# jolibrain/joliGEN

Measured on AMD Instinct MI355X. Metric: train images/sec at 256x256 (DDPM UNet step), higher is better.
Workload: dtype bf16; 1 GPU; palette_model DDPM, efficient UNet unet_mha ngf64 mults[1,2,4,8] res_blocks[2,2,2,2] mid-attn 16x32, 256x256, batch 32/GPU, inpainting synthetic masks, AdamW+EMA, iter_size 1 (example_ddpm_noglasses2glasses.json + SURVEY Appendix C overrides); global_batch=32, per_gpu_batch=32, image_size=256, efficient=True, parallelism=dp1, n_ranks_seen=1

## Files before the change

joligen_amd/csrc/capi.hip:

```cpp
#include "common.h"

extern "C" int jg_version(void) { return 100; }

extern "C" const char* jg_strerror(int code) {
  switch (code) {
    case JG_OK: return "ok";
    case JG_ERR_BAD_ARG: return "bad argument (null pointer, misaligned leading dimension or unsupported shape)";
    case JG_ERR_UNSUPPORTED: return "unsupported configuration";
    case JG_ERR_LAUNCH: return "HIP launch failed";
    default: return "unknown error";
  }
}

#include <atomic>
#include <cstdlib>
#include <cstring>
#include <mutex>

namespace {
struct TuneDef { const char* env; int dflt; };
const TuneDef kTune[JG_TUNE_COUNT] = {
    {"JG_HALO_CFG", 0}, {"JG_WGRAD_HALO_CFG", 0}, {"JG_CONV_VARIANT", 6}, {"JG_WGRAD_VARIANT", 4}, {"JG_SINKHORN_GENERIC", 0},
    {"JG_CONV1X1", 1}, {"JG_GN_REVERSE", 1}, {"JG_HALO_DBG", 0}, {"JG_PERSIST64", 1}, {"JG_HALO_PIPE", 1}, {"JG_WGRAD_PIPE", 1}, {"JG_CONV_SPLITK", 1}, {"JG_CONV_SMALL_TILE", 1}, {"JG_GN_FUSED", 1}, {"JG_GN_FUSED_CAP", 256}, {"JG_GN_FUSED_DBG", 0}, {"JG_GN_FUSED_SLEEP", 4}, {"JG_WGRAD_LDS_PAD", 0},
    {"JG_LN_BWD_CAP", 256}, {"JG_DW_BWD_CAP", 512}, {"JG_DW_BWD_PPT", 8}, {"JG_CONV_KXK", 1}, {"JG_CONV_RING", 1}, {"JG_WGRAD_DEEP", 1}, {"JG_WGRAD_SW", 0}, {"JG_DETERMINISTIC", 0}, {"JG_WGRAD_GROUP_BLOCKS", 1024}, {"JG_SGEMM_SPLIT", 0}, {"JG_WGRAD_BIG", 1}, {"JG_DW_RUN", 1}};
std::atomic<int> g_tune[JG_TUNE_COUNT];
std::once_flag g_tune_once;
void tune_init() {
  for (int i = 0; i < JG_TUNE_COUNT; ++i) {
    const char* e = getenv(kTune[i].env);
    g_tune[i].store(e ? atoi(e) : kTune[i].dflt, std::memory_order_relaxed);
  }
}
}

namespace {
thread_local const char* g_last_kernel = "";
}
void jg_note_kernel(const char* name) { g_last_kernel = name ? name : ""; }
extern "C" const char* jg_last_kernel(void) { return g_last_kernel; }

int jg_tune(int which) {
  std::call_once(g_tune_once, tune_init);
  return g_tune[which].load(std::memory_order_relaxed);
}

extern "C" int jg_set_tuning(const char* name, int value) {
  if (!name) return JG_ERR_BAD_ARG;
  std::call_once(g_tune_once, tune_init);
  for (int i = 0; i < JG_TUNE_COUNT; ++i)
    if (!strcmp(name, kTune[i].env)) {
      g_tune[i].store(value, std::memory_order_relaxed);
      return JG_OK;
    }
  return JG_ERR_BAD_ARG;
}

extern "C" int jg_get_tuning(const char* name) {
  if (!name) return -1;
  for (int i = 0; i < JG_TUNE_COUNT; ++i)
    if (!strcmp(name, kTune[i].env)) return jg_tune(i);
  return -1;
}
```

joligen_amd/csrc/common.h:

```cpp
#pragma once
#include <hip/hip_runtime.h>
#include <stdint.h>

#include "../../include/jg355.h"

typedef _Float16 f16_t;
typedef __bf16 bf16_t;
typedef _Float16 f16x8 __attribute__((ext_vector_type(8)));
typedef __bf16 bf16x8 __attribute__((ext_vector_type(8)));
typedef float f32x4 __attribute__((ext_vector_type(4)));

#define JG_WAVE 64

enum JgTune { JG_TUNE_HALO_CFG = 0, JG_TUNE_WGRAD_HALO_CFG, JG_TUNE_CONV_VARIANT, JG_TUNE_WGRAD_VARIANT, JG_TUNE_SINKHORN_GENERIC,
              JG_TUNE_CONV1X1, JG_TUNE_GN_REVERSE, JG_TUNE_HALO_DBG, JG_TUNE_PERSIST64, JG_TUNE_HALO_PIPE, JG_TUNE_WGRAD_PIPE, JG_TUNE_CONV_SPLITK, JG_TUNE_CONV_SMALL_TILE, JG_TUNE_GN_FUSED, JG_TUNE_GN_FUSED_CAP, JG_TUNE_GN_FUSED_DBG, JG_TUNE_GN_FUSED_SLEEP, JG_TUNE_WGRAD_LDS_PAD,
              JG_TUNE_LN_BWD_CAP, JG_TUNE_DW_BWD_CAP, JG_TUNE_DW_BWD_PPT, JG_TUNE_CONV_KXK, JG_TUNE_CONV_RING, JG_TUNE_WGRAD_DEEP, JG_TUNE_WGRAD_SW, JG_TUNE_DETERMINISTIC, JG_TUNE_WGRAD_GROUP_BLOCKS, JG_TUNE_SGEMM_SPLIT, JG_TUNE_WGRAD_BIG, JG_TUNE_DW_RUN, JG_TUNE_COUNT };
int jg_tune(int which);
void jg_note_kernel(const char* name);

#define JG_CHECK_LAUNCH()                          \
  do {                                             \
    if (hipGetLastError() != hipSuccess) return JG_ERR_LAUNCH; \
  } while (0)

template <typename T> __device__ __forceinline__ float to_f32(T v) { return (float)v; }
template <typename T> __device__ __forceinline__ T from_f32(float v) { return (T)v; }

template <typename T> __device__ __forceinline__ T bits_to(uint16_t b) { return __builtin_bit_cast(T, b); }
template <typename T> __device__ __forceinline__ uint16_t to_bits(T v) { return __builtin_bit_cast(uint16_t, v); }

template <typename T> __device__ __forceinline__ void unpack8(const uint4& v, float* f) {
  const uint32_t w[4] = {v.x, v.y, v.z, v.w};
#pragma unroll
  for (int i = 0; i < 4; ++i) {
    f[2 * i] = to_f32(bits_to<T>((uint16_t)(w[i] & 0xffffu)));
    f[2 * i + 1] = to_f32(bits_to<T>((uint16_t)(w[i] >> 16)));
  }
}
template <typename T> __device__ __forceinline__ uint4 pack8(const float* f) {
  uint32_t w[4];
#pragma unroll
  for (int i = 0; i < 4; ++i) {
    w[i] = (uint32_t)to_bits<T>(from_f32<T>(f[2 * i])) | ((uint32_t)to_bits<T>(from_f32<T>(f[2 * i + 1])) << 16);
  }
  return make_uint4(w[0], w[1], w[2], w[3]);
}
template <typename T> __device__ __forceinline__ uint2 pack4(float a, float b, float c, float d) {
  uint2 r;
  r.x = (uint32_t)to_bits<T>(from_f32<T>(a)) | ((uint32_t)to_bits<T>(from_f32<T>(b)) << 16);
  r.y = (uint32_t)to_bits<T>(from_f32<T>(c)) | ((uint32_t)to_bits<T>(from_f32<T>(d)) << 16);
  return r;
}
template <typename T> __device__ __forceinline__ void unpack4(const uint2& v, float* f) {
  f[0] = to_f32(bits_to<T>((uint16_t)(v.x & 0xffffu)));
  f[1] = to_f32(bits_to<T>((uint16_t)(v.x >> 16)));
  f[2] = to_f32(bits_to<T>((uint16_t)(v.y & 0xffffu)));
  f[3] = to_f32(bits_to<T>((uint16_t)(v.y >> 16)));
}

template <typename T> struct Mfma;
template <> struct Mfma<f16_t> {
  static __device__ __forceinline__ f32x4 run(const uint4& a, const uint4& b, f32x4 c) {
    return __builtin_amdgcn_mfma_f32_16x16x32_f16(__builtin_bit_cast(f16x8, a), __builtin_bit_cast(f16x8, b), c, 0, 0, 0);
  }
};
template <> struct Mfma<bf16_t> {
  static __device__ __forceinline__ f32x4 run(const uint4& a, const uint4& b, f32x4 c) {
    return __builtin_amdgcn_mfma_f32_16x16x32_bf16(__builtin_bit_cast(bf16x8, a), __builtin_bit_cast(bf16x8, b), c, 0, 0, 0);
  }
};

template <typename T> __device__ __forceinline__ uint4 ldg16(const T* ptr, bool ok) {
  uint4 v = *reinterpret_cast<const uint4*>(ptr);
  v.x = ok ? v.x : 0u;
  v.y = ok ? v.y : 0u;
  v.z = ok ? v.z : 0u;
  v.w = ok ? v.w : 0u;
  return v;
}

__device__ __forceinline__ float sigmoid_fast(float u) { return __builtin_amdgcn_rcpf(1.0f + __expf(-u)); }
__device__ __forceinline__ float silu_f(float u) { return u * sigmoid_fast(u); }
__device__ __forceinline__ float silu_grad_f(float u) {
  const float s = sigmoid_fast(u);
  return s * (1.0f + u * (1.0f - s));
}

template <int ACT> __device__ __forceinline__ float act_f(float u) {
  if (ACT == JG_ACT_SILU) return silu_f(u);
  if (ACT == JG_ACT_RELU) return fmaxf(u, 0.f);
  if (ACT == JG_ACT_LRELU) return u > 0.f ? u : 0.2f * u;
  return u;
}
template <int ACT> __device__ __forceinline__ float act_grad_f(float u) {
  if (ACT == JG_ACT_SILU) return silu_grad_f(u);
  if (ACT == JG_ACT_RELU) return u > 0.f ? 1.f : 0.f;
  if (ACT == JG_ACT_LRELU) return u > 0.f ? 1.f : 0.2f;
  return 1.f;
}
__device__ __forceinline__ float act_grad_rt(float u, int act) {
  return act == JG_ACT_SILU ? silu_grad_f(u) : act == JG_ACT_RELU ? (u > 0.f ? 1.f : 0.f) : act == JG_ACT_LRELU ? (u > 0.f ? 1.f : 0.2f) : 1.f;
}

#define JG_DISPATCH_ACT(act, ...)                          \
  do {                                                     \
    if ((act) == JG_ACT_SILU) { constexpr int ACT = JG_ACT_SILU; __VA_ARGS__ }        \
    else if ((act) == JG_ACT_RELU) { constexpr int ACT = JG_ACT_RELU; __VA_ARGS__ }   \
    else if ((act) == JG_ACT_LRELU) { constexpr int ACT = JG_ACT_LRELU; __VA_ARGS__ } \
    else { constexpr int ACT = JG_ACT_NONE; __VA_ARGS__ }                              \
  } while (0)

__device__ __forceinline__ float wave_sum(float v) {
#pragma unroll
  for (int o = 32; o > 0; o >>= 1) v += __shfl_xor(v, o);
  return v;
}
__device__ __forceinline__ float wave_max(float v) {
#pragma unroll
  for (int o = 32; o > 0; o >>= 1) v = fmaxf(v, __shfl_xor(v, o));
  return v;
}

#define JG_DISPATCH_DTYPE(dtype, ...)                 \
  do {                                                \
    if ((dtype) == JG_F16) {                          \
      typedef f16_t T;                                \
      __VA_ARGS__                                     \
    } else if ((dtype) == JG_BF16) {                  \
      typedef bf16_t T;                               \
      __VA_ARGS__                                     \
    } else {                                          \
      return JG_ERR_BAD_ARG;                          \
    }                                                 \
  } while (0)
```

joligen_amd/csrc/conv_p64.hip:

```cpp
#include "conv_params.h"
#include "conv_epilogue.h"

namespace {

constexpr int HW_ = 18;
constexpr int HALO_CH = HW_ * HW_ * 8;
constexpr int W_CH = 64 * 9 * 8;
constexpr int REGION = HALO_CH / 4;
constexpr int A_RD = (REGION + 63) / 64;

__device__ uint4 jg_p64_zero_page = {0u, 0u, 0u, 0u};

__device__ __forceinline__ void glds16(const void* gsrc, unsigned lds_dst) {
  unsigned keep;
  asm volatile("s_mov_b32 %0, m0\n\ts_mov_b32 m0, %2\n\ts_nop 0\n\tglobal_load_lds_dwordx4 %1, off\n\ts_mov_b32 m0, %0"
               : "=&s"(keep) : "v"(gsrc), "s"(lds_dst) : "memory");
}
template <int N> __device__ __forceinline__ void wait_vmcnt() { asm volatile("s_waitcnt vmcnt(%0)" ::"n"(N) : "memory"); }

struct TileRef { int b, oh0, ow0, sp; };

template <typename T>
__global__ __launch_bounds__(512, 1) void conv3x3_p64_kernel(ConvP p, int nsp, int Gs, int tilesN) {
  __shared__ uint4 sm[W_CH + 2 * HALO_CH + 16];
  const int tid = threadIdx.x, lane = tid & 63;
  const int wave = __builtin_amdgcn_readfirstlane(tid >> 6);
  const int g = wave >> 2, w = wave & 3;
  const int nb = blockIdx.x % tilesN, stream = blockIdx.x / tilesN;
  const int n0 = nb * 64;
  const int per = (nsp + Gs - 1) / Gs;
  const int ntl = stream * per < nsp ? (nsp - stream * per < per ? nsp - stream * per : per) : 0;
  const int tw = p.W >> 4, th = p.H >> 4;

  const T* __restrict__ x = (const T*)p.x;
  const T* __restrict__ wt = (const T*)p.w;
  const T* zp = reinterpret_cast<const T*>(&jg_p64_zero_page);
  typedef __attribute__((address_space(3))) char* lds_cptr;
  const unsigned lds0 = (unsigned)(size_t)(lds_cptr)(char*)&sm[0];
  char* smc = reinterpret_cast<char*>(&sm[0]);
  const unsigned hbyte = (W_CH + g * HALO_CH) * 16;

  auto tile_of = [&](int k) {
    TileRef t;
    t.sp = stream * per + k;
    t.ow0 = (t.sp % tw) << 4;
    t.oh0 = ((t.sp / tw) % th) << 4;
    t.b = t.sp / (tw * th);
    return t;
  };

  auto issue_halo = [&](const TileRef& t) {
    const long org = (((long)t.b * p.H + t.oh0) * p.W + t.ow0) * p.ldx;
    int lane_v = lane;
    asm volatile("" : "+v"(lane_v));
#pragma unroll
    for (int rd = 0; rd < A_RD; ++rd) {
      const int q = rd * 64 + lane_v;
      if (q < REGION) {
        const int pos = w * REGION + q;
        const int hp = pos >> 3, cpos = pos & 7;
        const int hy = (hp * 3641) >> 16, hx = hp - hy * HW_;
        const int kc = cpos ^ ((hx >> 1) & 7);
        const int ih = t.oh0 - 1 + hy, iw = t.ow0 - 1 + hx;
        const bool ok = (unsigned)ih < (unsigned)p.H && (unsigned)iw < (unsigned)p.W;
        const T* src = ok ? x + org + ((long)(hy - 1) * p.W + (hx - 1)) * p.ldx + kc * 8 : zp;
        glds16(src, lds0 + hbyte + (w * REGION + rd * 64) * 16);
      }
    }
  };

  {
    const int row = tid >> 3, cpos = tid & 7;
    const int kc = cpos ^ ((row >> 1) & 7);
    const bool ok = n0 + row < p.N;
    const T* src0 = wt + (long)(n0 + row) * p.ldw + kc * 8;
#pragma unroll
    for (int tap = 0; tap < 9; ++tap) glds16(ok ? src0 + tap * 64 : zp, lds0 + (tap * 512 + wave * 64) * 16);
  }
  if (g == 0 && ntl > 0) issue_halo(tile_of(0));

  const int l15 = lane & 15, lk = lane >> 4;
  float* sbias = reinterpret_cast<float*>(smc + (W_CH + 2 * HALO_CH) * 16);
  if (tid < 64) sbias[tid] = (p.bias && n0 + tid < p.N) ? p.bias[n0 + tid] : 0.f;

  int bfrag[4];
#pragma unroll
  for (int j = 0; j < 4; ++j) {
    const int row = j * 16 + l15;
    bfrag[j] = row * 128 + ((lk ^ ((row >> 1) & 7)) << 4);
  }
  int afrag[3];
#pragma unroll
  for (int s3 = 0; s3 < 3; ++s3) {
    const int hx = jg_pixperm(l15) + s3;
    afrag[s3] = ((w * 4) * HW_ + hx) * 128 + ((lk ^ ((hx >> 1) & 7)) << 4);
  }

  f32x4 acc[4][4];
  T* y = (T*)p.y;
  const T* res = (p.dbg & 32) ? nullptr : (const T*)p.res;
  uint2 rraw[4][4];
  auto load_res = [&](const TileRef& t) {
    const long m0 = ((long)t.b * p.H + t.oh0 + w * 4) * p.W + t.ow0 + jg_pixperm(l15);
#pragma unroll
    for (int i = 0; i < 4; ++i)
#pragma unroll
      for (int j = 0; j < 4; ++j)
        rraw[i][j] = *reinterpret_cast<const uint2*>(res + (m0 + (long)i * p.W) * p.ldres + n0 + lk * 4 + j * 16);
  };
  float s1[4][4], s2[4][4];
#pragma unroll
  for (int j = 0; j < 4; ++j)
#pragma unroll
    for (int q = 0; q < 4; ++q) s1[j][q] = s2[j][q] = 0.f;
  int stat_b = -1;
  auto flush_stats = [&]() {
    if (stat_b < 0 || !p.stats) return;
    float* dst = p.stats + (((long)stat_b * p.nslots + (blockIdx.x * 8 + wave) % p.nslots) * p.ldstats + n0) * 2;
#pragma unroll
    for (int j = 0; j < 4; ++j)
#pragma unroll
      for (int q = 0; q < 4; ++q) {
        float a = s1[j][q], b = s2[j][q];
#pragma unroll
        for (int o = 1; o < 16; o <<= 1) {
          a += __shfl_xor(a, o);
          b += __shfl_xor(b, o);
        }
        if (l15 == 0 && !(p.dbg & 64)) {
          atomicAdd(dst + (j * 16 + lk * 4 + q) * 2, a);
          atomicAdd(dst + (j * 16 + lk * 4 + q) * 2 + 1, b);
        }
        s1[j][q] = s2[j][q] = 0.f;
      }
  };
  wait_vmcnt<0>();
  __syncthreads();

  for (int ph = 0; ph <= ntl; ++ph) {
    if ((ph & 1) == g) {
      if (ph < ntl) {
        if (res) {
          if (ph < 2) load_res(tile_of(ph));
          const float rs = p.res_scale / p.alpha;
#pragma unroll
          for (int j = 0; j < 4; ++j)
#pragma unroll
            for (int i = 0; i < 4; ++i) {
              float rf[4];
              unpack4<T>(rraw[i][j], rf);
              acc[j][i] = (f32x4){rs * rf[0], rs * rf[1], rs * rf[2], rs * rf[3]};
            }
        } else {
#pragma unroll
          for (int j = 0; j < 4; ++j)
#pragma unroll
            for (int i = 0; i < 4; ++i) acc[j][i] = (f32x4){0.f, 0.f, 0.f, 0.f};
        }
        if (!(p.dbg & 2)) {
          const char* hb = smc + hbyte;
#pragma unroll
          for (int tap = 0; tap < 9; ++tap) {
            const int r = tap / 3, s3 = tap % 3;
            asm volatile("" ::: "memory");
#pragma unroll
            for (int sub = 0; sub < 2; ++sub) {
              if (sub) asm volatile("" ::: "memory");
              uint4 fa[4], fb[4];
              const int a0 = afrag[s3] ^ (sub * 64);
#pragma unroll
              for (int i = 0; i < 4; ++i) fa[i] = *reinterpret_cast<const uint4*>(hb + a0 + (i + r) * (HW_ * 128));
#pragma unroll
              for (int j = 0; j < 4; ++j) fb[j] = *reinterpret_cast<const uint4*>(smc + tap * 8192 + (bfrag[j] ^ (sub * 64)));
#pragma unroll
              for (int j = 0; j < 4; ++j)
#pragma unroll
                for (int i = 0; i < 4; ++i) acc[j][i] = Mfma<T>::run(fb[j], fa[i], acc[j][i]);
            }
          }
        }
      }
    } else {
      const int kt = ph - 1;
      const bool drain = kt >= 0 && kt < ntl && !(p.dbg & 1);
      const TileRef t = tile_of(drain ? kt : 0);
      const long mrow0 = ((long)t.b * p.H + t.oh0 + w * 4) * p.W + t.ow0 + jg_pixperm(l15);
      const bool fetch = ph + 1 < ntl && !(p.dbg & 4);
      if (fetch) issue_halo(tile_of(ph + 1));
      if (drain) {
        if (t.b != stat_b) {
          flush_stats();
          stat_b = t.b;
        }
        T* ybase = y + mrow0 * p.ldy + n0 + lk * 4;
        const long ystep = (long)p.W * p.ldy;
#pragma unroll
        for (int j = 0; j < 4; ++j) {
          const float4 bj = *reinterpret_cast<const float4*>(sbias + j * 16 + lk * 4);
          const float bq[4] = {bj.x, bj.y, bj.z, bj.w};
#pragma unroll
          for (int i = 0; i < 4; ++i) {
            float v[4];
#pragma unroll
            for (int q = 0; q < 4; ++q) v[q] = p.alpha * acc[j][i][q] + bq[q];
#pragma unroll
            for (int q = 0; q < 4; ++q) {
              s1[j][q] += v[q];
              s2[j][q] += v[q] * v[q];
            }
            if (!(p.dbg & 8)) *reinterpret_cast<uint2*>(ybase + i * ystep + j * 16) = pack4<T>(v[0], v[1], v[2], v[3]);
          }
        }
      }
      if (res && ph + 1 < ntl) {
        load_res(tile_of(ph + 1));
        wait_vmcnt<16>();
      } else {
        wait_vmcnt<0>();
      }
    }
    asm volatile("s_waitcnt lgkmcnt(0)" ::: "memory");
    __builtin_amdgcn_s_barrier();
  }
  flush_stats();
}

}

bool jg_conv_p64_try(int dtype, const ConvP& p0, int nbatch, hipStream_t st) {
  int mode = jg_tune(JG_TUNE_PERSIST64);
  if (!mode) return false;
  if (mode == 1 && p0.res) return false;
  if (mode == -1) mode = 1;
  ConvP p = p0;
  p.dbg = jg_tune(JG_TUNE_HALO_DBG);
  if (nbatch != 1 || p.R != 3 || p.S != 3 || p.pad != 1 || p.stride != 1 || p.out_f32) return false;
  if (p.Cin != 64 || p.N % 64 || (p.H & 15) || (p.W & 15) || p.H != p.Ho || p.W != p.Wo) return false;
  if (p.x_up || p.y_pool || p.res_up || p.reflect || (p.stats && p.stats_mode != 0) || p.alpha == 0.f) return false;
  if ((long)p.B * p.H * p.W * p.ldx >= (1L << 31) || (long)p.N * p.ldw >= (1L << 31)) return false;
  const int tilesN = p.N / 64;
  const int nsp = p.B * (p.H >> 4) * (p.W >> 4);
  if ((mode == 1 && nsp < 1024) || tilesN > 4) return false;
  int Gs = 256 / tilesN;
  if (mode >= 2 && Gs > mode) Gs = mode;
  if (Gs > nsp) Gs = nsp;
  const int grid = Gs * tilesN;
  jg_note_kernel("conv3x3_p64_kernel");
  if (dtype == JG_F16) hipLaunchKernelGGL((conv3x3_p64_kernel<f16_t>), dim3(grid), dim3(512), 0, st, p, nsp, Gs, tilesN);
  else if (dtype == JG_BF16) hipLaunchKernelGGL((conv3x3_p64_kernel<bf16_t>), dim3(grid), dim3(512), 0, st, p, nsp, Gs, tilesN);
  else return false;
  return true;
}
```

joligen_amd/csrc/mfma_pipe.h:

```cpp
#pragma once
#include <type_traits>
#include "common.h"

typedef unsigned u32x4 __attribute__((ext_vector_type(4)));

#define JG_MF_(MN, i) MN " %[c" #i "], %[b], %[a" #i "], %[c" #i "]\n\t"
#define JG_RD_(k) "ds_read_b128 %[d" #k "], %[p] offset:%[o" #k "]\n\t"
#define JG_C8_(c) [c0] "+v"(c[0]), [c1] "+v"(c[1]), [c2] "+v"(c[2]), [c3] "+v"(c[3]), [c4] "+v"(c[4]), [c5] "+v"(c[5]), [c6] "+v"(c[6]), [c7] "+v"(c[7])
#define JG_A8_(a) [a0] "v"(a[0]), [a1] "v"(a[1]), [a2] "v"(a[2]), [a3] "v"(a[3]), [a4] "v"(a[4]), [a5] "v"(a[5]), [a6] "v"(a[6]), [a7] "v"(a[7])
#define JG_C4_(c) [c0] "+v"(c[0]), [c1] "+v"(c[1]), [c2] "+v"(c[2]), [c3] "+v"(c[3])
#define JG_A4_(a) [a0] "v"(a[0]), [a1] "v"(a[1]), [a2] "v"(a[2]), [a3] "v"(a[3])

#define JG_G8R4_(MN)                                                                                                                  \
  asm volatile("s_waitcnt lgkmcnt(%[w])\n\t" JG_MF_(MN, 0) JG_RD_(0) JG_MF_(MN, 1) JG_MF_(MN, 2) JG_RD_(1) JG_MF_(MN, 3) JG_MF_(MN, 4)  \
               JG_RD_(2) JG_MF_(MN, 5) JG_MF_(MN, 6) JG_RD_(3) JG_MF_(MN, 7)                                                          \
               : JG_C8_(c), [d0] "=&v"(d0), [d1] "=&v"(d1), [d2] "=&v"(d2), [d3] "=&v"(d3)                                            \
               : JG_A8_(a), [b] "v"(b), [p] "v"(p), [w] "n"(W), [o0] "n"(O0), [o1] "n"(O1), [o2] "n"(O2), [o3] "n"(O3))
#define JG_G8R2_(MN)                                                                                                                  \
  asm volatile("s_waitcnt lgkmcnt(%[w])\n\t" JG_MF_(MN, 0) JG_MF_(MN, 1) JG_RD_(0) JG_MF_(MN, 2) JG_MF_(MN, 3) JG_MF_(MN, 4)            \
               JG_RD_(1) JG_MF_(MN, 5) JG_MF_(MN, 6) JG_MF_(MN, 7)                                                                    \
               : JG_C8_(c), [d0] "=&v"(d0), [d1] "=&v"(d1)                                                                            \
               : JG_A8_(a), [b] "v"(b), [p] "v"(p), [w] "n"(W), [o0] "n"(O0), [o1] "n"(O1))
#define JG_G8R0_(MN)                                                                                                                  \
  asm volatile("s_waitcnt lgkmcnt(%[w])\n\t" JG_MF_(MN, 0) JG_MF_(MN, 1) JG_MF_(MN, 2) JG_MF_(MN, 3) JG_MF_(MN, 4) JG_MF_(MN, 5)        \
               JG_MF_(MN, 6) JG_MF_(MN, 7)                                                                                            \
               : JG_C8_(c)                                                                                                            \
               : JG_A8_(a), [b] "v"(b), [w] "n"(W))
#define JG_G4R2_(MN)                                                                                                                  \
  asm volatile("s_waitcnt lgkmcnt(%[w])\n\t" JG_MF_(MN, 0) JG_RD_(0) JG_MF_(MN, 1) JG_MF_(MN, 2) JG_RD_(1) JG_MF_(MN, 3)               \
               : JG_C4_(c), [d0] "=&v"(d0), [d1] "=&v"(d1)                                                                            \
               : JG_A4_(a), [b] "v"(b), [p] "v"(p), [w] "n"(W), [o0] "n"(O0), [o1] "n"(O1))
#define JG_G4R0_(MN)                                                                                                                  \
  asm volatile("s_waitcnt lgkmcnt(%[w])\n\t" JG_MF_(MN, 0) JG_MF_(MN, 1) JG_MF_(MN, 2) JG_MF_(MN, 3)                                  \
               : JG_C4_(c)                                                                                                            \
               : JG_A4_(a), [b] "v"(b), [w] "n"(W))

#define JG_BY_TYPE_(BODY)                                       \
  if constexpr (std::is_same<T, bf16_t>::value) {               \
    BODY("v_mfma_f32_16x16x32_bf16");                           \
  } else {                                                      \
    BODY("v_mfma_f32_16x16x32_f16");                            \
  }

template <typename T, int W, int O0, int O1, int O2, int O3>
__device__ __forceinline__ void jg_g8r4(f32x4 (&c)[8], const u32x4& b, const u32x4 (&a)[8], u32x4& d0, u32x4& d1, u32x4& d2, u32x4& d3, unsigned p) {
  JG_BY_TYPE_(JG_G8R4_)
}
template <typename T, int W, int O0, int O1>
__device__ __forceinline__ void jg_g8r2(f32x4 (&c)[8], const u32x4& b, const u32x4 (&a)[8], u32x4& d0, u32x4& d1, unsigned p) {
  JG_BY_TYPE_(JG_G8R2_)
}
template <typename T, int W>
__device__ __forceinline__ void jg_g8r0(f32x4 (&c)[8], const u32x4& b, const u32x4 (&a)[8]) {
  JG_BY_TYPE_(JG_G8R0_)
}
template <typename T, int W, int O0, int O1>
__device__ __forceinline__ void jg_g4r2(f32x4 (&c)[4], const u32x4& b, const u32x4 (&a)[4], u32x4& d0, u32x4& d1, unsigned p) {
  JG_BY_TYPE_(JG_G4R2_)
}
template <typename T, int W>
__device__ __forceinline__ void jg_g4r0(f32x4 (&c)[4], const u32x4& b, const u32x4 (&a)[4]) {
  JG_BY_TYPE_(JG_G4R0_)
}

template <int O0, int O1, int O2, int O3>
__device__ __forceinline__ void jg_rd4(u32x4& d0, u32x4& d1, u32x4& d2, u32x4& d3, unsigned p) {
  asm volatile(JG_RD_(0) JG_RD_(1) JG_RD_(2) JG_RD_(3)
               : [d0] "=&v"(d0), [d1] "=&v"(d1), [d2] "=&v"(d2), [d3] "=&v"(d3)
               : [p] "v"(p), [o0] "n"(O0), [o1] "n"(O1), [o2] "n"(O2), [o3] "n"(O3));
}

template <typename T>
__device__ __forceinline__ void jg_mfma_pinned(f32x4& c, const uint4& a, const uint4& b) {
  const u32x4 av = {a.x, a.y, a.z, a.w}, bv = {b.x, b.y, b.z, b.w};
  if constexpr (std::is_same<T, bf16_t>::value) {
    asm volatile("s_nop 1\n\tv_mfma_f32_16x16x32_bf16 %0, %1, %2, %0" : "+v"(c) : "v"(av), "v"(bv) : "memory");
  } else {
    asm volatile("s_nop 1\n\tv_mfma_f32_16x16x32_f16 %0, %1, %2, %0" : "+v"(c) : "v"(av), "v"(bv) : "memory");
  }
}
```

Before: 660.3 images/sec.

## Software-pipeline LDS reads with MFMA in p64 conv and specialize epilogue

Adds a PIPE path to the 64-channel 3x3 conv kernel that interleaves ds_read_b128 fragment loads for the next substep between MFMA instructions through hand-written inline asm with double-buffered registers. It also templates the kernel on residual and stats presence so unused work compiles out, and precomputes halo offsets and edge masks once per thread instead of per tile. The epilogue now uses permlane16_swap to emit 16-byte stores and waits on partial vmcnt instead of draining all loads. Hand-tuned lgkmcnt counts and s_nop hazards add correctness risk, and there are now more kernel instantiations.

```diff
diff --git a/joligen_amd/csrc/capi.hip b/joligen_amd/csrc/capi.hip
--- a/joligen_amd/csrc/capi.hip
+++ b/joligen_amd/csrc/capi.hip
@@ -22,7 +22,7 @@
 const TuneDef kTune[JG_TUNE_COUNT] = {
     {"JG_HALO_CFG", 0}, {"JG_WGRAD_HALO_CFG", 0}, {"JG_CONV_VARIANT", 6}, {"JG_WGRAD_VARIANT", 4}, {"JG_SINKHORN_GENERIC", 0},
     {"JG_CONV1X1", 1}, {"JG_GN_REVERSE", 1}, {"JG_HALO_DBG", 0}, {"JG_PERSIST64", 1}, {"JG_HALO_PIPE", 1}, {"JG_WGRAD_PIPE", 1}, {"JG_CONV_SPLITK", 1}, {"JG_CONV_SMALL_TILE", 1}, {"JG_GN_FUSED", 1}, {"JG_GN_FUSED_CAP", 256}, {"JG_GN_FUSED_DBG", 0}, {"JG_GN_FUSED_SLEEP", 4}, {"JG_WGRAD_LDS_PAD", 0},
-    {"JG_LN_BWD_CAP", 256}, {"JG_DW_BWD_CAP", 512}, {"JG_DW_BWD_PPT", 8}, {"JG_CONV_KXK", 1}, {"JG_CONV_RING", 1}, {"JG_WGRAD_DEEP", 1}, {"JG_WGRAD_SW", 0}, {"JG_DETERMINISTIC", 0}, {"JG_WGRAD_GROUP_BLOCKS", 1024}, {"JG_SGEMM_SPLIT", 0}, {"JG_WGRAD_BIG", 1}, {"JG_DW_RUN", 1}};
+    {"JG_LN_BWD_CAP", 256}, {"JG_DW_BWD_CAP", 512}, {"JG_DW_BWD_PPT", 8}, {"JG_CONV_KXK", 1}, {"JG_CONV_RING", 1}, {"JG_WGRAD_DEEP", 1}, {"JG_WGRAD_SW", 0}, {"JG_DETERMINISTIC", 0}, {"JG_WGRAD_GROUP_BLOCKS", 1024}, {"JG_SGEMM_SPLIT", 0}, {"JG_WGRAD_BIG", 1}, {"JG_DW_RUN", 1}, {"JG_P64_PIPE", 1}};
 std::atomic<int> g_tune[JG_TUNE_COUNT];
 std::once_flag g_tune_once;
 void tune_init() {
diff --git a/joligen_amd/csrc/common.h b/joligen_amd/csrc/common.h
--- a/joligen_amd/csrc/common.h
+++ b/joligen_amd/csrc/common.h
@@ -14,7 +14,7 @@
 
 enum JgTune { JG_TUNE_HALO_CFG = 0, JG_TUNE_WGRAD_HALO_CFG, JG_TUNE_CONV_VARIANT, JG_TUNE_WGRAD_VARIANT, JG_TUNE_SINKHORN_GENERIC,
               JG_TUNE_CONV1X1, JG_TUNE_GN_REVERSE, JG_TUNE_HALO_DBG, JG_TUNE_PERSIST64, JG_TUNE_HALO_PIPE, JG_TUNE_WGRAD_PIPE, JG_TUNE_CONV_SPLITK, JG_TUNE_CONV_SMALL_TILE, JG_TUNE_GN_FUSED, JG_TUNE_GN_FUSED_CAP, JG_TUNE_GN_FUSED_DBG, JG_TUNE_GN_FUSED_SLEEP, JG_TUNE_WGRAD_LDS_PAD,
-              JG_TUNE_LN_BWD_CAP, JG_TUNE_DW_BWD_CAP, JG_TUNE_DW_BWD_PPT, JG_TUNE_CONV_KXK, JG_TUNE_CONV_RING, JG_TUNE_WGRAD_DEEP, JG_TUNE_WGRAD_SW, JG_TUNE_DETERMINISTIC, JG_TUNE_WGRAD_GROUP_BLOCKS, JG_TUNE_SGEMM_SPLIT, JG_TUNE_WGRAD_BIG, JG_TUNE_DW_RUN, JG_TUNE_COUNT };
+              JG_TUNE_LN_BWD_CAP, JG_TUNE_DW_BWD_CAP, JG_TUNE_DW_BWD_PPT, JG_TUNE_CONV_KXK, JG_TUNE_CONV_RING, JG_TUNE_WGRAD_DEEP, JG_TUNE_WGRAD_SW, JG_TUNE_DETERMINISTIC, JG_TUNE_WGRAD_GROUP_BLOCKS, JG_TUNE_SGEMM_SPLIT, JG_TUNE_WGRAD_BIG, JG_TUNE_DW_RUN, JG_TUNE_P64_PIPE, JG_TUNE_COUNT };
 int jg_tune(int which);
 void jg_note_kernel(const char* name);
 
diff --git a/joligen_amd/csrc/conv_p64.hip b/joligen_amd/csrc/conv_p64.hip
--- a/joligen_amd/csrc/conv_p64.hip
+++ b/joligen_amd/csrc/conv_p64.hip
@@ -1,5 +1,6 @@
 #include "conv_params.h"
 #include "conv_epilogue.h"
+#include "mfma_pipe.h"
 
 namespace {
 
@@ -20,7 +21,7 @@
 
 struct TileRef { int b, oh0, ow0, sp; };
 
-template <typename T>
+template <typename T, bool RES, bool STATS, bool PIPE>
 __global__ __launch_bounds__(512, 1) void conv3x3_p64_kernel(ConvP p, int nsp, int Gs, int tilesN) {
   __shared__ uint4 sm[W_CH + 2 * HALO_CH + 16];
   const int tid = threadIdx.x, lane = tid & 63;
@@ -49,21 +50,27 @@
     return t;
   };
 
+  unsigned hoff[A_RD];
+  unsigned hedge[2] = {0u, 0u};
+#pragma unroll
+  for (int rd = 0; rd < A_RD; ++rd) {
+    const int q = rd * 64 + lane;
+    const int pos = w * REGION + (q < REGION ? q : REGION - 1);
+    const int hp = pos >> 3, cpos = pos & 7;
+    const int hy = (hp * 3641) >> 16, hx = hp - hy * HW_;
+    const int kc = cpos ^ ((hx >> 1) & 7);
+    hoff[rd] = (unsigned)((((hy - 1) * p.W + (hx - 1)) * (int)p.ldx + kc * 8) * (int)sizeof(T));
+    const unsigned e = (hy == 0 ? 1u : 0u) | (hy == HW_ - 1 ? 2u : 0u) | (hx == 0 ? 4u : 0u) | (hx == HW_ - 1 ? 8u : 0u);
+    hedge[rd >> 3] |= e << ((rd & 7) * 4);
+  }
   auto issue_halo = [&](const TileRef& t) {
-    const long org = (((long)t.b * p.H + t.oh0) * p.W + t.ow0) * p.ldx;
-    int lane_v = lane;
-    asm volatile("" : "+v"(lane_v));
+    const unsigned org = (unsigned)(((((long)t.b * p.H + t.oh0) * p.W + t.ow0) * p.ldx) * (long)sizeof(T));
+    const unsigned em = (t.oh0 == 0 ? 1u : 0u) | (t.oh0 + 16 == p.H ? 2u : 0u) | (t.ow0 == 0 ? 4u : 0u) | (t.ow0 + 16 == p.W ? 8u : 0u);
 #pragma unroll
     for (int rd = 0; rd < A_RD; ++rd) {
-      const int q = rd * 64 + lane_v;
-      if (q < REGION) {
-        const int pos = w * REGION + q;
-        const int hp = pos >> 3, cpos = pos & 7;
-        const int hy = (hp * 3641) >> 16, hx = hp - hy * HW_;
-        const int kc = cpos ^ ((hx >> 1) & 7);
-        const int ih = t.oh0 - 1 + hy, iw = t.ow0 - 1 + hx;
-        const bool ok = (unsigned)ih < (unsigned)p.H && (unsigned)iw < (unsigned)p.W;
-        const T* src = ok ? x + org + ((long)(hy - 1) * p.W + (hx - 1)) * p.ldx + kc * 8 : zp;
+      if (rd < A_RD - 1 || lane < REGION - (A_RD - 1) * 64) {
+        const bool ok = ((hedge[rd >> 3] >> ((rd & 7) * 4)) & em) == 0;
+        const T* src = ok ? reinterpret_cast<const T*>(reinterpret_cast<const char*>(x) + (org + hoff[rd])) : zp;
         glds16(src, lds0 + hbyte + (w * REGION + rd * 64) * 16);
       }
     }
@@ -98,7 +105,7 @@
 
   f32x4 acc[4][4];
   T* y = (T*)p.y;
-  const T* res = (p.dbg & 32) ? nullptr : (const T*)p.res;
+  const T* res = (!RES || (p.dbg & 32)) ? nullptr : (const T*)p.res;
   uint2 rraw[4][4];
   auto load_res = [&](const TileRef& t) {
     const long m0 = ((long)t.b * p.H + t.oh0 + w * 4) * p.W + t.ow0 + jg_pixperm(l15);
@@ -109,19 +116,23 @@
         rraw[i][j] = *reinterpret_cast<const uint2*>(res + (m0 + (long)i * p.W) * p.ldres + n0 + lk * 4 + j * 16);
   };
   float s1[4][4], s2[4][4];
-#pragma unroll
-  for (int j = 0; j < 4; ++j)
-#pragma unroll
-    for (int q = 0; q < 4; ++q) s1[j][q] = s2[j][q] = 0.f;
+  if constexpr (STATS) {
+#pragma unroll
+    for (int j = 0; j < 4; ++j)
+#pragma unroll
+      for (int q = 0; q < 4; ++q) s1[j][q] = s2[j][q] = 0.f;
+  }
   int stat_b = -1;
+  const int stat_slot = STATS ? __builtin_amdgcn_readfirstlane((int)((blockIdx.x * 8 + wave) % (unsigned)p.nslots)) : 0;
   auto flush_stats = [&]() {
-    if (stat_b < 0 || !p.stats) return;
-    float* dst = p.stats + (((long)stat_b * p.nslots + (blockIdx.x * 8 + wave) % p.nslots) * p.ldstats + n0) * 2;
+    if (!STATS || stat_b < 0) return;
+    float* dst = p.stats + (((long)stat_b * p.nslots + stat_slot) * p.ldstats + n0) * 2;
 #pragma unroll
     for (int j = 0; j < 4; ++j)
 #pragma unroll
       for (int q = 0; q < 4; ++q) {
         float a = s1[j][q], b = s2[j][q];
+        asm volatile("" : "+v"(a), "+v"(b));
 #pragma unroll
         for (int o = 1; o < 16; o <<= 1) {
           a += __shfl_xor(a, o);
@@ -131,7 +142,6 @@
           atomicAdd(dst + (j * 16 + lk * 4 + q) * 2, a);
           atomicAdd(dst + (j * 16 + lk * 4 + q) * 2 + 1, b);
         }
-        s1[j][q] = s2[j][q] = 0.f;
       }
   };
   wait_vmcnt<0>();
@@ -140,7 +150,7 @@
   for (int ph = 0; ph <= ntl; ++ph) {
     if ((ph & 1) == g) {
       if (ph < ntl) {
-        if (res) {
+        if (RES && res) {
           if (ph < 2) load_res(tile_of(ph));
           const float rs = p.res_scale / p.alpha;
 #pragma unroll
@@ -157,7 +167,45 @@
 #pragma unroll
             for (int i = 0; i < 4; ++i) acc[j][i] = (f32x4){0.f, 0.f, 0.f, 0.f};
         }
-        if (!(p.dbg & 2)) {
+        if (PIPE && !(p.dbg & 2)) {
+          constexpr int RS = HW_ * 128;
+          u32x4 aP[4], bP[4], aQ[4], bQ[4];
+          const unsigned wb0 = lds0 + bfrag[0], hb0 = lds0 + hbyte;
+          auto abase = [&](int s) { return hb0 + (afrag[(s >> 1) % 3] ^ ((s & 1) * 64)); };
+          auto bbase = [&](int s) { return ((wb0 - lds0) ^ ((s & 1) * 64)) + lds0 + ((s >> 1) >= 5 ? 5 * 8192 : 0); };
+          auto substep = [&](auto sc, u32x4 (&ca)[4], u32x4 (&cb)[4], u32x4 (&na)[4], u32x4 (&nb)[4]) {
+            constexpr int s = decltype(sc)::value;
+            if constexpr (s < 17) {
+              constexpr int ntap = (s + 1) >> 1, nr = ntap / 3, WO = (ntap >= 5 ? ntap - 5 : ntap) * 8192;
+              const unsigned pa = abase(s + 1), pb = bbase(s + 1);
+              jg_g4r3<T, 3, WO, nr * RS, (nr + 1) * RS>(acc[0], cb[0], ca, nb[0], na[0], na[1], pb, pa, pa);
+              jg_g4r3<T, 5, (nr + 2) * RS, (nr + 3) * RS, WO + 2048>(acc[1], cb[1], ca, na[2], na[3], nb[1], pa, pa, pb);
+              jg_g4r2<T, 7, WO + 4096, WO + 6144>(acc[2], cb[2], ca, nb[2], nb[3], pb);
+              jg_g4r0<T, 8>(acc[3], cb[3], ca);
+            } else {
+              jg_g4r0<T, 3>(acc[0], cb[0], ca);
+              jg_g4r0<T, 2>(acc[1], cb[1], ca);
+              jg_g4r0<T, 1>(acc[2], cb[2], ca);
+              jg_g4r0<T, 0>(acc[3], cb[3], ca);
+            }
+          };
+          {
+            const unsigned pa = abase(0), pb = bbase(0);
+            jg_rd1<0>(bP[0], pb);
+            jg_rd4<0, RS, 2 * RS, 3 * RS>(aP[0], aP[1], aP[2], aP[3], pa);
+            jg_rd1<2048>(bP[1], pb);
+            jg_rd1<4096>(bP[2], pb);
+            jg_rd1<6144>(bP[3], pb);
+          }
+          asm volatile("s_nop 1"
+                       : "+v"(acc[0][0]), "+v"(acc[0][1]), "+v"(acc[0][2]), "+v"(acc[0][3]), "+v"(acc[1][0]), "+v"(acc[1][1]), "+v"(acc[1][2]),
+                         "+v"(acc[1][3]), "+v"(acc[2][0]), "+v"(acc[2][1]), "+v"(acc[2][2]), "+v"(acc[2][3]), "+v"(acc[3][0]), "+v"(acc[3][1]),
+                         "+v"(acc[3][2]), "+v"(acc[3][3]));
+#define JG_P64_SS_(s) substep(std::integral_constant<int, s>{}, aP, bP, aQ, bQ); substep(std::integral_constant<int, s + 1>{}, aQ, bQ, aP, bP);
+          JG_P64_SS_(0) JG_P64_SS_(2) JG_P64_SS_(4) JG_P64_SS_(6) JG_P64_SS_(8) JG_P64_SS_(10) JG_P64_SS_(12) JG_P64_SS_(14) JG_P64_SS_(16)
+#undef JG_P64_SS_
+          asm volatile("s_nop 15\n\ts_nop 15" ::: "memory");
+        } else if (!(p.dbg & 2)) {
           const char* hb = smc + hbyte;
 #pragma unroll
           for (int tap = 0; tap < 9; ++tap) {
@@ -187,37 +235,67 @@
       const long mrow0 = ((long)t.b * p.H + t.oh0 + w * 4) * p.W + t.ow0 + jg_pixperm(l15);
       const bool fetch = ph + 1 < ntl && !(p.dbg & 4);
       if (fetch) issue_halo(tile_of(ph + 1));
+      bool flushed = false;
       if (drain) {
-        if (t.b != stat_b) {
+        if (STATS && t.b != stat_b) {
+          flushed = stat_b >= 0;
           flush_stats();
           stat_b = t.b;
         }
-        T* ybase = y + mrow0 * p.ldy + n0 + lk * 4;
+        if constexpr (STATS) {
+#pragma unroll
+          for (int j = 0; j < 4; ++j)
+#pragma unroll
+            for (int q = 0; q < 4; ++q) {
+              s1[j][q] = flushed ? 0.f : s1[j][q];
+              s2[j][q] = flushed ? 0.f : s2[j][q];
+            }
+        }
+        T* ybase = y + mrow0 * p.ldy + n0 + ((lk & 1) ? 16 + (lk - 1) * 4 : lk * 4);
         const long ystep = (long)p.W * p.ldy;
 #pragma unroll
-        for (int j = 0; j < 4; ++j) {
-          const float4 bj = *reinterpret_cast<const float4*>(sbias + j * 16 + lk * 4);
-          const float bq[4] = {bj.x, bj.y, bj.z, bj.w};
+        for (int jp = 0; jp < 4; jp += 2) {
+          float bq[2][4];
+#pragma unroll
+          for (int h = 0; h < 2; ++h) {
+            const float4 bj = *reinterpret_cast<const float4*>(sbias + (jp + h) * 16 + lk * 4);
+            bq[h][0] = bj.x, bq[h][1] = bj.y, bq[h][2] = bj.z, bq[h][3] = bj.w;
+          }
 #pragma unroll
           for (int i = 0; i < 4; ++i) {
-            float v[4];
-#pragma unroll
-            for (int q = 0; q < 4; ++q) v[q] = p.alpha * acc[j][i][q] + bq[q];
-#pragma unroll
-            for (int q = 0; q < 4; ++q) {
-              s1[j][q] += v[q];
-              s2[j][q] += v[q] * v[q];
-            }
-            if (!(p.dbg & 8)) *reinterpret_cast<uint2*>(ybase + i * ystep + j * 16) = pack4<T>(v[0], v[1], v[2], v[3]);
+            uint2 pk[2];
+#pragma unroll
+            for (int h = 0; h < 2; ++h) {
+              const int j = jp + h;
+              float v[4];
+#pragma unroll
+              for (int q = 0; q < 4; ++q) {
+                v[q] = p.alpha * acc[j][i][q] + bq[h][q];
+                asm("" : "+v"(v[q]));
+              }
+              if constexpr (STATS) {
+#pragma unroll
+                for (int q = 0; q < 4; ++q) {
+                  s1[j][q] += v[q];
+                  s2[j][q] += v[q] * v[q];
+                }
+              }
+              pk[h] = pack4<T>(v[0], v[1], v[2], v[3]);
+            }
+            const auto sx = __builtin_amdgcn_permlane16_swap(pk[0].x, pk[1].x, false, false);
+            const auto sy = __builtin_amdgcn_permlane16_swap(pk[0].y, pk[1].y, false, false);
+            if (!(p.dbg & 8)) *reinterpret_cast<uint4*>(ybase + i * ystep + jp * 16) = make_uint4(sx[0], sy[0], sx[1], sy[1]);
           }
         }
       }
-      if (res && ph + 1 < ntl) {
-        load_res(tile_of(ph + 1));
-        wait_vmcnt<16>();
-      } else {
-        wait_vmcnt<0>();
-      }
+      const bool stored = drain && !(p.dbg & 8);
+      const bool rows = RES && res && ph + 1 < ntl;
+      if (rows) load_res(tile_of(ph + 1));
+      if (flushed) wait_vmcnt<0>();
+      else if (stored && rows) wait_vmcnt<8 + 16>();
+      else if (stored) wait_vmcnt<8>();
+      else if (rows) wait_vmcnt<16>();
+      else wait_vmcnt<0>();
     }
     asm volatile("s_waitcnt lgkmcnt(0)" ::: "memory");
     __builtin_amdgcn_s_barrier();
@@ -235,9 +313,11 @@
   ConvP p = p0;
   p.dbg = jg_tune(JG_TUNE_HALO_DBG);
   if (nbatch != 1 || p.R != 3 || p.S != 3 || p.pad != 1 || p.stride != 1 || p.out_f32) return false;
+  if (((size_t)p.y & 15) || (p.ldy & 7)) return false;
   if (p.Cin != 64 || p.N % 64 || (p.H & 15) || (p.W & 15) || p.H != p.Ho || p.W != p.Wo) return false;
   if (p.x_up || p.y_pool || p.res_up || p.reflect || (p.stats && p.stats_mode != 0) || p.alpha == 0.f) return false;
   if ((long)p.B * p.H * p.W * p.ldx >= (1L << 31) || (long)p.N * p.ldw >= (1L << 31)) return false;
+  if ((long)(HW_ + 1) * p.W * p.ldx >= (1L << 30)) return false;
   const int tilesN = p.N / 64;
   const int nsp = p.B * (p.H >> 4) * (p.W >> 4);
   if ((mode == 1 && nsp < 1024) || tilesN > 4) return false;
@@ -245,9 +325,24 @@
   if (mode >= 2 && Gs > mode) Gs = mode;
   if (Gs > nsp) Gs = nsp;
   const int grid = Gs * tilesN;
+  if (dtype != JG_F16 && dtype != JG_BF16) return false;
+  const bool pipe = jg_tune(JG_TUNE_P64_PIPE) != 0;
   jg_note_kernel("conv3x3_p64_kernel");
-  if (dtype == JG_F16) hipLaunchKernelGGL((conv3x3_p64_kernel<f16_t>), dim3(grid), dim3(512), 0, st, p, nsp, Gs, tilesN);
-  else if (dtype == JG_BF16) hipLaunchKernelGGL((conv3x3_p64_kernel<bf16_t>), dim3(grid), dim3(512), 0, st, p, nsp, Gs, tilesN);
-  else return false;
+#define JG_P64_LAUNCH_(T, RES, STATS, PIPE) \
+  hipLaunchKernelGGL((conv3x3_p64_kernel<T, RES, STATS, PIPE>), dim3(grid), dim3(512), 0, st, p, nsp, Gs, tilesN)
+#define JG_P64_BY_(T)                                                                  \
+  do {                                                                                 \
+    if (p.res) {                                                                       \
+      if (p.stats) { if (pipe) JG_P64_LAUNCH_(T, true, true, true); else JG_P64_LAUNCH_(T, true, true, false); }       \
+      else { if (pipe) JG_P64_LAUNCH_(T, true, false, true); else JG_P64_LAUNCH_(T, true, false, false); }             \
+    } else {                                                                           \
+      if (p.stats) { if (pipe) JG_P64_LAUNCH_(T, false, true, true); else JG_P64_LAUNCH_(T, false, true, false); }     \
+      else { if (pipe) JG_P64_LAUNCH_(T, false, false, true); else JG_P64_LAUNCH_(T, false, false, false); }           \
+    }                                                                                  \
+  } while (0)
+  if (dtype == JG_F16) JG_P64_BY_(f16_t);
+  else JG_P64_BY_(bf16_t);
+#undef JG_P64_BY_
+#undef JG_P64_LAUNCH_
   return true;
 }
diff --git a/joligen_amd/csrc/mfma_pipe.h b/joligen_amd/csrc/mfma_pipe.h
--- a/joligen_amd/csrc/mfma_pipe.h
+++ b/joligen_amd/csrc/mfma_pipe.h
@@ -35,6 +35,12 @@
                : JG_C4_(c)                                                                                                            \
                : JG_A4_(a), [b] "v"(b), [w] "n"(W))
 
+#define JG_RDP_(k) "ds_read_b128 %[d" #k "], %[p" #k "] offset:%[o" #k "]\n\t"
+#define JG_G4R3_(MN)                                                                                                                  \
+  asm volatile("s_waitcnt lgkmcnt(%[w])\n\t" JG_MF_(MN, 0) JG_RDP_(0) JG_MF_(MN, 1) JG_RDP_(1) JG_MF_(MN, 2) JG_RDP_(2) JG_MF_(MN, 3)  \
+               : JG_C4_(c), [d0] "=&v"(d0), [d1] "=&v"(d1), [d2] "=&v"(d2)                                                            \
+               : JG_A4_(a), [b] "v"(b), [p0] "v"(p0), [p1] "v"(p1), [p2] "v"(p2), [w] "n"(W), [o0] "n"(O0), [o1] "n"(O1), [o2] "n"(O2))
+
 #define JG_BY_TYPE_(BODY)                                       \
   if constexpr (std::is_same<T, bf16_t>::value) {               \
     BODY("v_mfma_f32_16x16x32_bf16");                           \
@@ -58,6 +64,10 @@
 __device__ __forceinline__ void jg_g4r2(f32x4 (&c)[4], const u32x4& b, const u32x4 (&a)[4], u32x4& d0, u32x4& d1, unsigned p) {
   JG_BY_TYPE_(JG_G4R2_)
 }
+template <typename T, int W, int O0, int O1, int O2>
+__device__ __forceinline__ void jg_g4r3(f32x4 (&c)[4], const u32x4& b, const u32x4 (&a)[4], u32x4& d0, u32x4& d1, u32x4& d2, unsigned p0, unsigned p1, unsigned p2) {
+  JG_BY_TYPE_(JG_G4R3_)
+}
 template <typename T, int W>
 __device__ __forceinline__ void jg_g4r0(f32x4 (&c)[4], const u32x4& b, const u32x4 (&a)[4]) {
   JG_BY_TYPE_(JG_G4R0_)
@@ -70,6 +80,11 @@
                : [p] "v"(p), [o0] "n"(O0), [o1] "n"(O1), [o2] "n"(O2), [o3] "n"(O3));
 }
 
+template <int O0>
+__device__ __forceinline__ void jg_rd1(u32x4& d0, unsigned p) {
+  asm volatile(JG_RD_(0) : [d0] "=&v"(d0) : [p] "v"(p), [o0] "n"(O0));
+}
+
 template <typename T>
 __device__ __forceinline__ void jg_mfma_pinned(f32x4& c, const uint4& a, const uint4& b) {
   const u32x4 av = {a.x, a.y, a.z, a.w}, bv = {b.x, b.y, b.z, b.w};
```

Measured after the change: 663.7 images/sec, median of 6. Within noise of the previous version (+0.5%).
